# daniabib/ComfyUI_ProPainter_Nodes

Measured on NVIDIA H100. Metric: inpainted frames/sec at 640x360, 80-frame subvideo, higher is better.
Workload: dtype f16

## Files before the change

comfyui_propainter_nodes_b200/csrc/conv_epilogue.cuh:

```cuda
#pragma once
#include "conv_igemm.cuh"
#include "wgmma_ops.cuh"

namespace ppconv {

template <int ACT, bool ACC = false, int N>
__device__ __forceinline__ void act16_t(float (&v)[N], float slope) {
#pragma unroll
  for (int i = 0; i < N; ++i) {
    if (ACT == PP_ACT_RELU) v[i] = fmaxf(v[i], 0.f);
    else if (ACT == PP_ACT_LRELU) v[i] = v[i] > 0.f ? v[i] : v[i] * slope;
    else if (ACT == PP_ACT_SIGMOID) v[i] = ppx::sigmoidf_(v[i]);
    else if (ACT == PP_ACT_TANH) v[i] = ACC ? ppx::tanh_acc(v[i]) : tanhf(v[i]);
    else if (ACT == PP_ACT_GELU) v[i] = ppx::gelu_erf(v[i]);
  }
}
template <bool ACC = false, int N>
__device__ __forceinline__ void act16(float (&v)[N], int act, float slope) {
  switch (act) {
    case PP_ACT_RELU: act16_t<PP_ACT_RELU, ACC>(v, slope); break;
    case PP_ACT_LRELU: act16_t<PP_ACT_LRELU, ACC>(v, slope); break;
    case PP_ACT_SIGMOID: act16_t<PP_ACT_SIGMOID, ACC>(v, slope); break;
    case PP_ACT_TANH: act16_t<PP_ACT_TANH, ACC>(v, slope); break;
    case PP_ACT_GELU: act16_t<PP_ACT_GELU, ACC>(v, slope); break;
    default: break;
  }
}

__device__ __forceinline__ void load16(const __half* src, int nvalid, bool vec, float (&r)[16]) {
  if (vec && nvalid == 16) {
    const uint4 a = reinterpret_cast<const uint4*>(src)[0], b = reinterpret_cast<const uint4*>(src)[1];
    const __half2* ha = reinterpret_cast<const __half2*>(&a);
    const __half2* hb = reinterpret_cast<const __half2*>(&b);
#pragma unroll
    for (int i = 0; i < 4; ++i) {
      const float2 fa = __half22float2(ha[i]), fb = __half22float2(hb[i]);
      r[2 * i] = fa.x; r[2 * i + 1] = fa.y; r[8 + 2 * i] = fb.x; r[8 + 2 * i + 1] = fb.y;
    }
  } else {
#pragma unroll
    for (int i = 0; i < 16; ++i) r[i] = i < nvalid ? __half2float(src[i]) : 0.f;
  }
}
__device__ __forceinline__ void store16(__half* dst, int nvalid, bool vec, const float (&v)[16]) {
  if (vec && nvalid == 16) {
    __align__(16) __half2 h[8];
#pragma unroll
    for (int i = 0; i < 8; ++i) h[i] = __floats2half2_rn(v[2 * i], v[2 * i + 1]);
    reinterpret_cast<uint4*>(dst)[0] = reinterpret_cast<uint4*>(h)[0];
    reinterpret_cast<uint4*>(dst)[1] = reinterpret_cast<uint4*>(h)[1];
  } else {
#pragma unroll
    for (int i = 0; i < 16; ++i)
      if (i < nvalid) dst[i] = __float2half_rn(v[i]);
  }
}

__device__ __forceinline__ void conv_epilogue16(const PPConvParams& p, const uint32_t (&raw)[16], long long mrow, int g,
                                                int ng0, int epi, bool vec) {
    const int nvalid = min(16, p.Cout_g - ng0);
    float v[16];
#pragma unroll
    for (int i = 0; i < 16; ++i) v[i] = __uint_as_float(raw[i]);
    if (p.bias != nullptr) {
      const float* bp = p.bias + g * p.Cout_g + ng0;
      if (vec && nvalid == 16) {
#pragma unroll
        for (int i = 0; i < 4; ++i) {
          const float4 b4 = __ldg(reinterpret_cast<const float4*>(bp) + i);
          v[4 * i] += b4.x; v[4 * i + 1] += b4.y; v[4 * i + 2] += b4.z; v[4 * i + 3] += b4.w;
        }
      } else {
#pragma unroll
        for (int i = 0; i < 16; ++i)
          if (i < nvalid) v[i] += __ldg(bp + i);
      }
    }
    if (epi == PP_EPI_STD) {
      act16(v, p.act1, p.slope);
      if (p.scale != 1.f) {
#pragma unroll
        for (int i = 0; i < 16; ++i) v[i] *= p.scale;
      }
      if (p.aux0 != nullptr) {
        float r[16];
        load16(p.aux0 + mrow * p.aux0_cstride + p.aux0_coff + ng0, nvalid, vec, r);
#pragma unroll
        for (int i = 0; i < 16; ++i) v[i] += r[i];
      }
      act16(v, p.act2, p.slope);
      const long long o = mrow * p.out_cstride + p.out_coff + (long long)g * p.out_gstep + ng0;
      if (p.out_fp32) {
        float* dst = reinterpret_cast<float*>(p.out) + o;
        if (vec && nvalid == 16) {
#pragma unroll
          for (int i = 0; i < 4; ++i)
            reinterpret_cast<float4*>(dst)[i] = make_float4(v[4 * i], v[4 * i + 1], v[4 * i + 2], v[4 * i + 3]);
        } else {
#pragma unroll
          for (int i = 0; i < 16; ++i)
            if (i < nvalid) dst[i] = v[i];
        }
      } else {
        store16(reinterpret_cast<__half*>(p.out) + o, nvalid, vec, v);
      }
    } else if (epi == PP_EPI_GRU_ZR) {
      const int half_c = p.Cout_g >> 1;
      act16_t<PP_ACT_SIGMOID>(v, 0.f);
      if (ng0 < half_c) {
        store16(reinterpret_cast<__half*>(p.out) + mrow * p.out_cstride + p.out_coff + ng0, nvalid, vec, v);
      } else {
        const int c = ng0 - half_c;
        float h[16];
        load16(p.aux0 + mrow * p.aux0_cstride + p.aux0_coff + c, nvalid, vec, h);
#pragma unroll
        for (int i = 0; i < 16; ++i) v[i] *= h[i];
        store16(p.out2 + mrow * p.out2_cstride + p.out2_coff + c, nvalid, vec, v);
      }
    } else {
      float h[16], z[16];
      load16(p.aux0 + mrow * p.aux0_cstride + p.aux0_coff + ng0, nvalid, vec, h);
      load16(p.aux1 + mrow * p.aux1_cstride + p.aux1_coff + ng0, nvalid, vec, z);
      act16_t<PP_ACT_TANH>(v, 0.f);
#pragma unroll
      for (int i = 0; i < 16; ++i) v[i] = (1.f - z[i]) * h[i] + z[i] * v[i];
      store16(reinterpret_cast<__half*>(p.out) + mrow * p.out_cstride + p.out_coff + ng0, nvalid, vec, v);
    }
}


template <int BN>
__device__ __forceinline__ void stage_bias(const PPConvParams& p, float* bs, int goff, int n0, int t128) {
  const int c0 = 2 * t128, n = goff + n0 + c0;
  float2 bv = make_float2(0.f, 0.f);
  if (p.bias != nullptr && c0 < BN) {
    if (n0 + c0 < p.Cout_g) bv.x = __ldg(p.bias + n);
    if (n0 + c0 + 1 < p.Cout_g) bv.y = __ldg(p.bias + n + 1);
  }
  if (c0 < BN) *reinterpret_cast<float2*>(bs + c0) = bv;
}

template <int PW>
__device__ __forceinline__ int frag_stg_off(int r, int c) {
  return r * PW * 2 + ((((c & (PW - 1)) >> 3) ^ ((r * PW * 2 >> 7) & (PW / 8 - 1))) << 4) + (c & 7) * 2;
}

template <int MB, int BN, int PW, int PANEL, int EPI, int ACT1>
__device__ __forceinline__ void frag_epilogue(const PPConvParams& p, const float (&acc)[MB][BN / 2], uint8_t* so,
                                              const uint8_t* zb, const float* bs, bool has_aux, bool r_tile, int P,
                                              int t128) {
  const bool has_bias = p.bias != nullptr;
  const float scale = p.scale, slope = p.slope;
  const int act2 = p.act2;
  const int fr = 16 * (t128 >> 5) + ((t128 & 31) >> 2), fc = 2 * (t128 & 3);
#pragma unroll
  for (int b = 0; b < MB; ++b) {
    const int r = 64 * b + fr;
#pragma unroll
    for (int j = 0; j < BN / 8; ++j) {
      const int col = 8 * j + fc;
      if (EPI == PP_EPI_GRU_H && col / PW != P) continue;
      const int off = (col / PW) * PANEL + frag_stg_off<PW>(r, col);
      __half2* lo = reinterpret_cast<__half2*>(so + off);
      __half2* hi = reinterpret_cast<__half2*>(so + off + 8 * PW * 2);
      const float2 bias = *reinterpret_cast<const float2*>(bs + col);
      float v[4] = {acc[b][4 * j], acc[b][4 * j + 1], acc[b][4 * j + 2], acc[b][4 * j + 3]};
      float a[4] = {0.f, 0.f, 0.f, 0.f};
      if (has_aux) {
        const float2 a0 = __half22float2(*lo), a1 = __half22float2(*hi);
        a[0] = a0.x; a[1] = a0.y; a[2] = a1.x; a[3] = a1.y;
      }
      if (has_bias) {
        v[0] += bias.x; v[1] += bias.y; v[2] += bias.x; v[3] += bias.y;
      }
      if constexpr (EPI == PP_EPI_STD) {
        act16_t<ACT1>(v, slope);
        if (scale != 1.f) {
#pragma unroll
          for (int i = 0; i < 4; ++i) v[i] *= scale;
        }
        if (has_aux) {
#pragma unroll
          for (int i = 0; i < 4; ++i) v[i] += a[i];
        }
        if (act2 != PP_ACT_NONE) act16(v, act2, slope);
      } else if constexpr (EPI == PP_EPI_GRU_ZR) {
        act16_t<PP_ACT_SIGMOID>(v, 0.f);
        if (r_tile) {
#pragma unroll
          for (int i = 0; i < 4; ++i) v[i] *= a[i];
        }
      } else {
        const int zoff = frag_stg_off<PW>(r, col);
        const float2 z0 = __half22float2(*reinterpret_cast<const __half2*>(zb + zoff));
        const float2 z1 = __half22float2(*reinterpret_cast<const __half2*>(zb + zoff + 8 * PW * 2));
        const float z[4] = {z0.x, z0.y, z1.x, z1.y};
        act16_t<PP_ACT_TANH>(v, 0.f);
#pragma unroll
        for (int i = 0; i < 4; ++i) v[i] = (1.f - z[i]) * a[i] + z[i] * v[i];
      }
      *lo = __floats2half2_rn(v[0], v[1]);
      *hi = __floats2half2_rn(v[2], v[3]);
    }
  }
}

__device__ __forceinline__ void load16_split(const float* src, int lo, int nvalid, bool vec, float (&r)[16]) {
  if (vec && nvalid == 16) {
#pragma unroll
    for (int i = 0; i < 4; ++i) {
      const float4 h = reinterpret_cast<const float4*>(src)[i], l = reinterpret_cast<const float4*>(src + lo)[i];
      r[4 * i] = h.x + l.x; r[4 * i + 1] = h.y + l.y; r[4 * i + 2] = h.z + l.z; r[4 * i + 3] = h.w + l.w;
    }
  } else {
#pragma unroll
    for (int i = 0; i < 16; ++i) r[i] = i < nvalid ? src[i] + src[lo + i] : 0.f;
  }
}
__device__ __forceinline__ void store16_split(float* dst, int lo, int nvalid, bool vec, const float (&v)[16]) {
  float h[16], l[16];
#pragma unroll
  for (int i = 0; i < 16; ++i) { h[i] = ppx::tf32_rna(v[i]); l[i] = v[i] - h[i]; }
  if (vec && nvalid == 16) {
#pragma unroll
    for (int i = 0; i < 4; ++i) {
      reinterpret_cast<float4*>(dst)[i] = make_float4(h[4 * i], h[4 * i + 1], h[4 * i + 2], h[4 * i + 3]);
      reinterpret_cast<float4*>(dst + lo)[i] = make_float4(l[4 * i], l[4 * i + 1], l[4 * i + 2], l[4 * i + 3]);
    }
  } else {
#pragma unroll
    for (int i = 0; i < 16; ++i)
      if (i < nvalid) { dst[i] = h[i]; dst[lo + i] = l[i]; }
  }
}

__device__ __forceinline__ void conv_epilogue16_split(const PPConvParams& p, const float (&acc)[16], long long mrow, int g,
                                                      int ng0, bool vec) {
  const int nvalid = min(16, p.Cout_g - ng0);
  float v[16];
#pragma unroll
  for (int i = 0; i < 16; ++i) v[i] = acc[i];
  if (p.bias != nullptr) {
    const float* bp = p.bias + g * p.Cout_g + ng0;
#pragma unroll
    for (int i = 0; i < 16; ++i)
      if (i < nvalid) v[i] += __ldg(bp + i);
  }
  const float* aux0 = reinterpret_cast<const float*>(p.aux0);
  const float* aux1 = reinterpret_cast<const float*>(p.aux1);
  float* out = reinterpret_cast<float*>(p.out);
  if (p.epi == PP_EPI_STD) {
    act16<true>(v, p.act1, p.slope);
    if (p.scale != 1.f) {
#pragma unroll
      for (int i = 0; i < 16; ++i) v[i] *= p.scale;
    }
    if (aux0 != nullptr) {
      float r[16];
      load16_split(aux0 + mrow * p.aux0_cstride + p.aux0_coff + ng0, p.aux0_lo, nvalid, vec, r);
#pragma unroll
      for (int i = 0; i < 16; ++i) v[i] += r[i];
    }
    act16<true>(v, p.act2, p.slope);
    float* dst = out + mrow * p.out_cstride + p.out_coff + (long long)g * p.out_gstep + ng0;
    if (p.out_fp32) {
      if (vec && nvalid == 16) {
#pragma unroll
        for (int i = 0; i < 4; ++i)
          reinterpret_cast<float4*>(dst)[i] = make_float4(v[4 * i], v[4 * i + 1], v[4 * i + 2], v[4 * i + 3]);
      } else {
#pragma unroll
        for (int i = 0; i < 16; ++i)
          if (i < nvalid) dst[i] = v[i];
      }
    } else {
      store16_split(dst, p.out_lo, nvalid, vec, v);
    }
  } else if (p.epi == PP_EPI_GRU_ZR) {
    const int half_c = p.Cout_g >> 1;
    act16_t<PP_ACT_SIGMOID, true>(v, 0.f);
    if (ng0 < half_c) {
      store16_split(out + mrow * p.out_cstride + p.out_coff + ng0, p.out_lo, nvalid, vec, v);
    } else {
      const int c = ng0 - half_c;
      float h[16];
      load16_split(aux0 + mrow * p.aux0_cstride + p.aux0_coff + c, p.aux0_lo, nvalid, vec, h);
#pragma unroll
      for (int i = 0; i < 16; ++i) v[i] *= h[i];
      store16_split(reinterpret_cast<float*>(p.out2) + mrow * p.out2_cstride + p.out2_coff + c, p.out2_lo, nvalid, vec, v);
    }
  } else {
    float h[16], z[16];
    load16_split(aux0 + mrow * p.aux0_cstride + p.aux0_coff + ng0, p.aux0_lo, nvalid, vec, h);
    load16_split(aux1 + mrow * p.aux1_cstride + p.aux1_coff + ng0, p.aux1_lo, nvalid, vec, z);
    act16_t<PP_ACT_TANH, true>(v, 0.f);
#pragma unroll
    for (int i = 0; i < 16; ++i) v[i] = (1.f - z[i]) * h[i] + z[i] * v[i];
    store16_split(out + mrow * p.out_cstride + p.out_coff + ng0, p.out_lo, nvalid, vec, v);
  }
}

constexpr int STG_LD = 40;
constexpr int STG_BYTES = 64 * STG_LD * 4;

template <int N, class Emit>
__device__ __forceinline__ void drain_acc(const float (&acc)[N / 2], float* stg, int t128, int bar_id, Emit&& emit) {
  const int wrow = 16 * (t128 >> 5) + ((t128 & 31) >> 2), wcol = 2 * (t128 & 3);
#pragma unroll 1
  for (int c0 = 0; c0 < N; c0 += 32) {
#pragma unroll
    for (int cc = 0; cc < N; cc += 32) {
      if (cc == c0) {
#pragma unroll
        for (int j = 0; j < 4; ++j) {
          if (cc + 8 * j < N) {
            const int i = (cc / 8 + j) * 4;
            *reinterpret_cast<float2*>(stg + wrow * STG_LD + 8 * j + wcol) = make_float2(acc[i], acc[i + 1]);
            *reinterpret_cast<float2*>(stg + (wrow + 8) * STG_LD + 8 * j + wcol) = make_float2(acc[i + 2], acc[i + 3]);
          }
        }
      }
    }
    ppx::named_bar(bar_id, 128);
    const int c = c0 + 16 * (t128 & 1);
    if (c < N) emit(stg + (t128 >> 1) * STG_LD + 16 * (t128 & 1), t128 >> 1, c);
    ppx::named_bar(bar_id, 128);
  }
}

template <bool SPLIT = false, int EPI = -1>
__device__ __forceinline__ void epilogue_from_stage(const PPConvParams& p, const float* src, long long mrow, int g, int ng0) {
  if constexpr (SPLIT) {
    float acc[16];
#pragma unroll
    for (int i = 0; i < 16; i += 4) {
      const float4 v = *reinterpret_cast<const float4*>(src + i);
      acc[i] = v.x; acc[i + 1] = v.y; acc[i + 2] = v.z; acc[i + 3] = v.w;
    }
// ... 47 lines not shown
```

comfyui_propainter_nodes_b200/csrc/conv_gemm.cu:

```cuda
#include <string.h>

#include "conv_epilogue.cuh"
#include "conv_igemm.cuh"

namespace {

constexpr int NUM_THREADS = 384;
constexpr int NUM_CONSUMERS = 256;
constexpr int WARP_PRODUCER = 8;
constexpr int STAGE_BYTES = 48 * 1024;
constexpr int STAGES = 3;
constexpr int OUT_BYTES = 64 * 1024;
constexpr int BIAS_BYTES = 2 * 256 * 4;
constexpr int SMEM_BYTES = 1024 + STAGES * STAGE_BYTES + OUT_BYTES + 1024 + BIAS_BYTES;

struct GemmParams {
  PPConvParams c;
  CUtensorMap tmap_a[PP_MAX_SEGS];
  CUtensorMap tmap_out;
  CUtensorMap tmap_res;
  int m_tiles, n_tiles, chunks;
  int debug;
};

struct Smem {
  uint8_t* stages;
  uint8_t* out;
  uint64_t *full, *empty, *res;
  float* bias;
};
__device__ __forceinline__ Smem gemm_smem() {
  uint8_t* base = ppx::dyn_smem_1024();
  Smem m;
  m.stages = base;
  m.out = base + STAGES * STAGE_BYTES;
  m.full = reinterpret_cast<uint64_t*>(m.out + OUT_BYTES);
  m.empty = m.full + STAGES;
  m.res = m.empty + STAGES;
  m.bias = reinterpret_cast<float*>(m.out + OUT_BYTES + 1024);
  return m;
}

template <int MB, int BN>
__device__ __forceinline__ void gemm_tile(const GemmParams& h, const Smem& m, int tile, int& s, uint32_t& ph, uint32_t& rph,
                                          int wg, int t128) {
  using namespace ppx;
  const PPConvParams& p = h.c;
  constexpr int A_BYTES = 128 * MB * 128;
  constexpr int WG_ROWS = 64 * MB;
  constexpr int PANEL = 128 * MB * 128;
  const int n0 = (tile % h.n_tiles) * BN;
  const int m0 = (tile / h.n_tiles) * (128 * MB);
  float acc[MB][BN / 2];
  int prev = -1;
  for (int c = 0; c < h.chunks; ++c) {
    mbar_wait(&m.full[s], ph);
    const uint32_t a = smem_u32(m.stages + s * STAGE_BYTES);
    uint64_t adesc[MB];
#pragma unroll
    for (int b = 0; b < MB; ++b) adesc[b] = gmma_desc_sw128_kmajor(a + (wg * MB + b) * 64 * 128);
    const uint64_t bdesc = gmma_desc_sw128_kmajor(a + A_BYTES);
    wgmma_fence();
#pragma unroll
    for (int k = 0; k < 4; ++k)
#pragma unroll
      for (int b = 0; b < MB; ++b) wgmma_f16<BN>(acc[b], adesc[b] + 2 * k, bdesc + 2 * k, (c | k) != 0 ? 1u : 0u);
    wgmma_commit();
    wgmma_wait<1>();
    if (prev >= 0) mbar_arrive(&m.empty[prev]);
    prev = s;
    if (++s == STAGES) { s = 0; ph ^= 1; }
  }
  wgmma_wait<0>();
#pragma unroll
  for (int b = 0; b < MB; ++b) wgmma_fence_acc(acc[b]);
  mbar_arrive(&m.empty[prev]);
  if (h.debug & 1) return;

  const int bar_id = 2 + wg, row0 = m0 + wg * WG_ROWS;
  const int npanel = (min(BN, p.Cout_g - n0) + 63) / 64;
  uint8_t* so = m.out + wg * WG_ROWS * 128;
  const bool issuer = t128 == 0;
  float* bs = m.bias + wg * 256;
  ppconv::stage_bias<BN>(p, bs, 0, n0, t128);
  if (issuer) tma_store_wait_read<0>();
  named_bar(bar_id, 128);
  const bool has_res = p.aux0 != nullptr;
  if (has_res) {
    if (issuer) {
      mbar_arrive_expect_tx(&m.res[wg], (uint32_t)(npanel * WG_ROWS * 128));
      for (int pnl = 0; pnl < npanel; ++pnl) tma_load_2d(smem_u32(so + pnl * PANEL), &h.tmap_res, n0 + pnl * 64, row0, &m.res[wg]);
    }
    mbar_wait(&m.res[wg], rph);
    rph ^= 1;
  }
  auto epilogue = [&](auto act1) {
    ppconv::frag_epilogue<MB, BN, 64, PANEL, PP_EPI_STD, decltype(act1)::value>(p, acc, so, nullptr, bs, has_res, false, 0,
                                                                                t128);
  };
  switch (p.act1) {
    case PP_ACT_RELU: epilogue(ppconv::IntC<PP_ACT_RELU>{}); break;
    case PP_ACT_LRELU: epilogue(ppconv::IntC<PP_ACT_LRELU>{}); break;
    case PP_ACT_SIGMOID: epilogue(ppconv::IntC<PP_ACT_SIGMOID>{}); break;
    case PP_ACT_TANH: epilogue(ppconv::IntC<PP_ACT_TANH>{}); break;
    case PP_ACT_GELU: epilogue(ppconv::IntC<PP_ACT_GELU>{}); break;
    default: epilogue(ppconv::IntC<PP_ACT_NONE>{}); break;
  }
  fence_proxy_async();
  named_bar(bar_id, 128);
  if (issuer) {
    for (int pnl = 0; pnl < npanel; ++pnl) tma_store_2d(&h.tmap_out, smem_u32(so + pnl * PANEL), n0 + pnl * 64, row0);
    tma_store_commit();
  }
}

template <int MB>
__global__ void __launch_bounds__(NUM_THREADS, 1) conv_gemm_kernel(const __grid_constant__ GemmParams h) {
  using namespace ppx;
  constexpr int BN = 256 / MB;
  constexpr int A_BYTES = 128 * MB * 128;
  const Smem m = gemm_smem();
  const PPConvParams& p = h.c;
  const int tid = threadIdx.x, warp = tid >> 5;
  const int total_tiles = h.m_tiles * h.n_tiles;
  if (tid == 0) {
    for (int s = 0; s < STAGES; ++s) { mbar_init(&m.full[s], 1); mbar_init(&m.empty[s], NUM_CONSUMERS); }
    mbar_init(&m.res[0], 1);
    mbar_init(&m.res[1], 1);
    mbar_fence_init();
  }
  __syncthreads();
  asm volatile("griddepcontrol.wait;" ::: "memory");
  asm volatile("griddepcontrol.launch_dependents;" ::: "memory");

  if (warp < 8) setmaxnreg_inc<232>();
  else setmaxnreg_dec<40>();
  if (warp < 8) {
    const int wg = tid >> 7, t128 = tid & 127;
    int s = 0;
    uint32_t ph = 0, rph = 0;
    for (int tile = blockIdx.x; tile < total_tiles; tile += gridDim.x) gemm_tile<MB, BN>(h, m, tile, s, ph, rph, wg, t128);
    if (t128 == 0) tma_store_wait<0>();
  } else if (warp == WARP_PRODUCER) {
    if (elect_one()) {
      int s = 0;
      uint32_t ph = 0;
      for (int tile = blockIdx.x; tile < total_tiles; tile += gridDim.x) {
        const int n0 = (tile % h.n_tiles) * BN;
        const int m0 = (tile / h.n_tiles) * (128 * MB);
        const uint32_t b_bytes = (uint32_t)(min(BN, p.Cout_g_pad - n0) * 128);
        for (int c = 0; c < h.chunks; ++c) {
          const int ci = c * 64;
          const int q = pp_seg_of(p, ci);
          mbar_wait(&m.empty[s], ph ^ 1);
          mbar_arrive_expect_tx(&m.full[s], (uint32_t)A_BYTES + b_bytes);
          const uint32_t dst = smem_u32(m.stages + s * STAGE_BYTES);
          tma_load_4d(dst, &h.tmap_a[q], ci - p.seg[q].cbegin, m0, 0, 0, &m.full[s]);
          bulk_g2s(dst + A_BYTES, p.wpacked + ((long long)c * p.Cout_g_pad + n0) * 64, b_bytes, &m.full[s]);
          if (++s == STAGES) { s = 0; ph ^= 1; }
        }
      }
    }
  }
}

int gemm_mb(const PPConvParams& p) { return p.Cout_g_pad <= 128 && p.M_total >= 256 ? 2 : 1; }

long long gemm_tiles(const PPConvParams& p, int mb) {
  return pp_ceil_div64(p.M_total, 128 * mb) * pp_ceil_div(p.Cout_g_pad, 256 / mb);
}

}

int pp_conv_gemm_eligible(const PPConvParams& p) {
  if (p.kh != 1 || p.kw != 1 || p.sh != 1 || p.sw != 1 || p.ph != 0 || p.pw != 0 || p.pad_replicate) return 0;
  if (p.groups != 1 || p.split || p.epi != PP_EPI_STD || p.out_fp32 || p.M_total < 128) return 0;
  if (!pp_conv_segs_chunked(p, true)) return 0;
  if (!aligned16(p.out, p.out_cstride, p.out_coff)) return 0;
  if (p.aux0 != nullptr && !aligned16(p.aux0, p.aux0_cstride, p.aux0_coff)) return 0;
  if (p.bias != nullptr && (reinterpret_cast<uintptr_t>(p.bias) & 7) != 0) return 0;
  int num_sms = 0;
  if (pp_num_sms(&num_sms) != PP_OK || gemm_tiles(p, gemm_mb(p)) < num_sms) return 0;
  return pp_tmap_supported() ? 1 : 0;
}

int pp_launch_conv_gemm(const PPConvParams& pin, cudaStream_t stream) {
  static bool attr_set = false;
  if (!attr_set) {
    PP_CUDA_CHECK(cudaFuncSetAttribute(conv_gemm_kernel<1>, cudaFuncAttributeMaxDynamicSharedMemorySize, SMEM_BYTES));
    PP_CUDA_CHECK(cudaFuncSetAttribute(conv_gemm_kernel<2>, cudaFuncAttributeMaxDynamicSharedMemorySize, SMEM_BYTES));
    attr_set = true;
  }
  GemmParams h;
  memset(&h, 0, sizeof(h));
  h.c = pin;
  const PPConvParams& p = h.c;
  const int mb = gemm_mb(p);
  h.m_tiles = (int)pp_ceil_div64(p.M_total, 128 * mb);
  h.n_tiles = pp_ceil_div(p.Cout_g_pad, 256 / mb);
  h.chunks = pp_ceil_div(p.Cin, 64);
  PP_REQUIRE((long long)h.m_tiles * h.n_tiles < (1LL << 31), "conv_gemm: too many tiles");
  h.debug = pp_conv_noepi();
  PP_TRY(pp_conv_input_tmaps(p, 128 * mb, 1, true, h.tmap_a));
  PP_TRY(pp_tmap_2d_f16(&h.tmap_out, static_cast<const __half*>(p.out) + p.out_coff, p.Cout_g, p.M_total, p.out_cstride, 64 * mb));
  if (p.aux0 != nullptr)
    PP_TRY(pp_tmap_2d_f16(&h.tmap_res, p.aux0 + p.aux0_coff, p.Cout_g, p.M_total, p.aux0_cstride, 64 * mb));
  int num_sms = 0;
  PP_TRY(pp_num_sms(&num_sms));
  return pp_conv_launch(mb == 2 ? conv_gemm_kernel<2> : conv_gemm_kernel<1>, h, min(h.m_tiles * h.n_tiles, num_sms),
                        NUM_THREADS, SMEM_BYTES, stream);
}
```

comfyui_propainter_nodes_b200/csrc/conv_halo.cu:

```cuda
#include <cuda.h>
#include <stdlib.h>
#include <string.h>

#include <memory>

#include "conv_epilogue.cuh"
#include "conv_igemm.cuh"
#include "dcn_sample.cuh"

namespace {

constexpr int NUM_THREADS = 384;
constexpr int NUM_EPI_THREADS = 256;
constexpr int WARP_A = 8, WARP_B = 9;
constexpr int MAX_SA = 4, MAX_SB = 8;
constexpr int SMEM_BUDGET = 186 * 1024;
constexpr int SMEM_MAX = 227 * 1024;
constexpr int SMEM_ALIGN_SLACK = 1024;
constexpr int BAR_BLOCK_BYTES = 1024;
constexpr int DRAIN_EPI_BYTES = 2 * ppconv::STG_BYTES;

struct HaloLayer {
  PPConvParams c;
  CUtensorMap tmap[PP_MAX_SEGS];
// ... 91 lines not shown
__device__ __forceinline__ void halo_tap_group(int tn, float (&acc)[MB][BN / 2], uint64_t (&adesc)[MB], uint64_t bdesc,
                                               uint32_t& accum, int& kx, int kw, uint32_t step_x, uint32_t step_row,
                                               uint32_t tap16) {
  using namespace ppx;
  if constexpr (NT > 1) {
    if (tn < NT) {
      halo_tap_group<BN, MB, NT - 1, TF32>(tn, acc, adesc, bdesc, accum, kx, kw, step_x, step_row, tap16);
      return;
    }
  }
  wgmma_fence();
#pragma unroll
  for (int tt = 0; tt < NT; ++tt) halo_tap<BN, MB, TF32>(acc, adesc, bdesc, accum, kx, kw, step_x, step_row, tap16);
  wgmma_commit();
}

template <int BN, int MB, int NT, bool TF32, class BeforeWait>
__device__ __forceinline__ void halo_mainloop(const HaloLayer& h, const HaloSmem& m, Ring& ra, Ring& rb, int wg,
                                              float (&acc)[MB][BN / 2], BeforeWait&& before_wait) {
  using namespace ppx;
  const PPConvParams& p = h.c;
  const int taps = p.kh * p.kw;
  const uint32_t sbo = h.flat ? 1024u : (uint32_t)h.BW * 128;
  const uint32_t step_x = (uint32_t)p.dw * 8;
  const uint32_t step_row = (uint32_t)(p.dh * h.BW - (p.kw - 1) * p.dw) * 8;
  const uint32_t tap16 = (uint32_t)p.BN * 8;
  const int kw = p.kw;
  uint32_t aoff[MB];
#pragma unroll
  for (int b = 0; b < MB; ++b) aoff[b] = MB == 2 ? wg * h.sub_bytes + b * 8 * sbo : wg * 8 * sbo;
  uint32_t accum = 0;
  int pend_a = -1, pend_b = -1;
  for (int c = 0; c < h.chunks; ++c) {
    mbar_wait(&m.a_full[ra.s], ra.ph);
    uint64_t adesc[MB];
#pragma unroll
    for (int b = 0; b < MB; ++b) adesc[b] = gmma_desc_sw128_kmajor(smem_u32(m.a + ra.s * m.a_stage_bytes) + aoff[b], sbo);
    int kx = 0;
    for (int tap0 = 0; tap0 < taps; tap0 += h.tps) {
      mbar_wait(&m.b_full[rb.s], rb.ph);
      const uint64_t bdesc = gmma_desc_sw128_kmajor(smem_u32(m.b + rb.s * m.b_stage_bytes));
      halo_tap_group<BN, MB, NT, TF32>(min(h.tps, taps - tap0), acc, adesc, bdesc, accum, kx, kw, step_x, step_row, tap16);
      wgmma_wait<1>();
      if (pend_b >= 0) mbar_arrive(&m.b_empty[pend_b]);
      if (pend_a >= 0) mbar_arrive(&m.a_empty[pend_a]);
      pend_b = rb.s;
      pend_a = tap0 + h.tps >= taps ? ra.s : -1;
      if (++rb.s == m.SB) { rb.s = 0; rb.ph ^= 1; }
    }
    if (++ra.s == m.SA) { ra.s = 0; ra.ph ^= 1; }
  }
  before_wait();
  wgmma_wait<0>();
#pragma unroll
  for (int b = 0; b < MB; ++b) wgmma_fence_acc(acc[b]);
  if (pend_b >= 0) mbar_arrive(&m.b_empty[pend_b]);
  if (pend_a >= 0) mbar_arrive(&m.a_empty[pend_a]);
}

template <int BN, int MB, int NT, bool TF32 = false, bool PROG = false>
__device__ __forceinline__ void halo_tile(const HaloLayer& h, int tile, const HaloSmem& m, Ring& ra, Ring& rb, float* stg,
                                          int wg, int t128) {
  const PPConvParams& p = h.c;
  const TileCoord t = decode_tile(h, tile);
  const int n0 = t.n_idx * p.BN;
  const int bnt = min(p.BN, p.Cout_g_pad - n0);
  float acc[MB][BN / 2];
  halo_mainloop<BN, MB, NT, TF32>(h, m, ra, rb, wg, acc, [] {});

  const bool skip = (h.debug & 1) != 0;
#pragma unroll
  for (int b = 0; b < MB; ++b) {
    const int sub = MB == 2 ? wg : 0, rbase = MB == 2 ? 64 * b : 64 * wg;
    ppconv::drain_acc<BN>(acc[b], stg, t128, 4 + wg, [&](const float* src, int r64, int cc) {
      const int r = rbase + r64;
      bool mvalid;
      long long mrow;
      if (h.flat) {
        mrow = ((long long)t.tx * h.MT + sub) * 128 + r;
        mvalid = mrow < p.M_total;
      } else {
        const int oy = t.ty * 16 + (r >> 3), ox = t.tx * (8 * h.MT) + 8 * sub + (r & 7);
        mvalid = oy < p.OH && ox < p.OW;
        mrow = ((long long)t.img * p.OH + oy) * p.OW + ox;
      }
      if (!mvalid || skip || cc >= bnt || n0 + cc >= p.Cout_g) return;
      ppconv::epilogue_from_stage<TF32, PROG ? PP_EPI_STD : -1>(p, src, mrow, t.g, n0 + cc);
    });
  }
}

__host__ __device__ constexpr int halo_panel_width(int bn) { return bn % 64 == 0 ? 64 : bn % 32 == 0 ? 32 : 16; }
__host__ __device__ constexpr int halo_out_stage_bytes(int mt, int bn) { return 2 * 64 * mt * bn * 2; }
__host__ __device__ constexpr int halo_out_bias_bytes(int bn) { return (2 * bn * 4 + 1023) / 1024 * 1024; }
__host__ __device__ constexpr int halo_out_z_bytes(int mt, int bn) { return 2 * 64 * mt * halo_panel_width(bn) * 2; }
__host__ __device__ constexpr int halo_tma_region_bytes(int mt, int bn, bool gru_h) {
  return halo_out_stage_bytes(mt, bn) + halo_out_bias_bytes(bn) + (gru_h ? halo_out_z_bytes(mt, bn) : 0);
}
__host__ __device__ inline int halo_epi_bytes(const HaloParams& h) {
  return h.tma_out ? halo_tma_region_bytes(h.MT, h.c.BN, h.c.epi == PP_EPI_GRU_H) : DRAIN_EPI_BYTES;
}
__device__ __forceinline__ uint64_t* halo_out_bar(const HaloSmem& m, int wg) { return m.spare + 1 + wg; }

template <int BN, int MB, int NT>
__device__ __forceinline__ void halo_tile_tma(const HaloParams& h, int tile, const HaloSmem& m, Ring& ra, Ring& rb,
                                              uint32_t& xph, int wg, int t128) {
  using namespace ppx;
  const PPConvParams& p = h.c;
  constexpr int PW = halo_panel_width(BN);
  constexpr int PANEL = 64 * MB * PW * 2;
  const TileCoord t = decode_tile(h, tile);
  const int n0 = t.n_idx * BN;
  const int epi = p.epi;
  const int half_c = p.Cout_g >> 1;
  const bool r_tile = epi == PP_EPI_GRU_ZR && n0 >= half_c;
  const bool has_aux = epi == PP_EPI_STD ? p.aux0 != nullptr : (epi == PP_EPI_GRU_H || r_tile);
  const int npanel = (min(BN, p.Cout_g - n0) + PW - 1) / PW;
  uint8_t* so = m.epi + wg * (64 * MB * BN * 2);
  float* bs = reinterpret_cast<float*>(m.epi + halo_out_stage_bytes(MB, BN)) + wg * BN;
  uint8_t* zb = m.epi + halo_out_stage_bytes(MB, BN) + halo_out_bias_bytes(BN) + wg * PANEL;
  uint64_t* xbar = halo_out_bar(m, wg);
  int x0, y0, img;
  if (h.flat) {
    x0 = MB == 2 ? (t.tx * 2 + wg) * 128 : t.tx * 128 + 64 * wg; y0 = 0; img = 0;
  } else {
    x0 = t.tx * (8 * MB) + (MB == 2 ? 8 * wg : 0); y0 = t.ty * 16 + (MB == 2 ? 0 : 8 * wg); img = t.img;
  }
  const int aux_c = r_tile ? n0 - half_c : n0;
  const bool issuer = t128 == 0;
  const bool skip = (h.debug & 1) != 0;
  float acc[MB][BN / 2];
  halo_mainloop<BN, MB, NT, false>(h, m, ra, rb, wg, acc, [&] {
    if (issuer && has_aux && !skip) {
      tma_store_wait_read<0>();
      const int nz = epi == PP_EPI_GRU_H ? 1 : 0;
      mbar_arrive_expect_tx(xbar, (uint32_t)((npanel + nz) * PANEL));
      for (int pn = 0; pn < npanel; ++pn)
        tma_load_4d(smem_u32(so + pn * PANEL), &h.tm_aux0, aux_c + pn * PW, x0, y0, img, xbar);
      if (nz) tma_load_4d(smem_u32(zb), &h.tm_aux1, n0, x0, y0, img, xbar);
    }
  });
  if (skip) return;

  ppconv::stage_bias<BN>(p, bs, t.g * p.Cout_g, n0, t128);
  const int bar_id = 4 + wg;
  if (issuer && !has_aux) tma_store_wait_read<0>();
  named_bar(bar_id, 128);
  if (has_aux) {
    mbar_wait(xbar, xph);
    xph ^= 1;
  }
  using ppconv::IntC;
  auto epilogue = [&](auto kind, auto act1, bool aux, int P) {
    ppconv::frag_epilogue<MB, BN, PW, PANEL, decltype(kind)::value, decltype(act1)::value>(p, acc, so, zb, bs, aux, r_tile,
                                                                                           P, t128);
  };
  if (epi == PP_EPI_STD) {
    switch (p.act1) {
      case PP_ACT_RELU: epilogue(IntC<PP_EPI_STD>{}, IntC<PP_ACT_RELU>{}, has_aux, 0); break;
      case PP_ACT_LRELU: epilogue(IntC<PP_EPI_STD>{}, IntC<PP_ACT_LRELU>{}, has_aux, 0); break;
      default: epilogue(IntC<PP_EPI_STD>{}, IntC<PP_ACT_NONE>{}, has_aux, 0); break;
    }
  } else if (epi == PP_EPI_GRU_ZR) {
    epilogue(IntC<PP_EPI_GRU_ZR>{}, IntC<PP_ACT_NONE>{}, r_tile, 0);
  } else {
#pragma unroll 1
    for (int pn = 0; pn < npanel; ++pn) {
      if (pn > 0) {
        named_bar(bar_id, 128);
        if (issuer) {
          mbar_arrive_expect_tx(xbar, (uint32_t)PANEL);
          tma_load_4d(smem_u32(zb), &h.tm_aux1, n0 + pn * PW, x0, y0, img, xbar);
        }
        mbar_wait(xbar, xph);
        xph ^= 1;
      }
      epilogue(IntC<PP_EPI_GRU_H>{}, IntC<PP_ACT_NONE>{}, true, pn);
    }
  }
  fence_proxy_async();
  named_bar(bar_id, 128);
  if (issuer) {
    const CUtensorMap* tm = r_tile ? &h.tm_out2 : &h.tm_out;
    const int c0 = r_tile ? n0 - half_c : t.g * p.out_gstep + n0;
    for (int pn = 0; pn < npanel; ++pn) tma_store_4d(tm, smem_u32(so + pn * PANEL), c0 + pn * PW, x0, y0, img);
    tma_store_commit();
  }
}

template <class F>
__device__ __forceinline__ void with_tile_shape(int mt, int bn, F&& f) {
  if (mt == 2) ppconv::with_tile_width<128>(bn, [&](auto n) { f(n, ppconv::IntC<2>{}); });
  else ppconv::with_tile_width<256>(bn, [&](auto n) { f(n, ppconv::IntC<1>{}); });
}

__device__ __forceinline__ void halo_smem_init_barriers(const HaloSmem& m) {
  using namespace ppx;
  for (int s = 0; s < m.SA; ++s) { mbar_init(&m.a_full[s], 1); mbar_init(&m.a_empty[s], NUM_EPI_THREADS); }
  for (int s = 0; s < m.SB; ++s) { mbar_init(&m.b_full[s], 1); mbar_init(&m.b_empty[s], NUM_EPI_THREADS); }
  mbar_fence_init();
}

__device__ __forceinline__ void halo_produce_patches(const HaloLayer& h, const HaloSmem& m, Ring& r) {
  using namespace ppx;
  const PPConvParams& p = h.c;
  const int total_tiles = halo_total_tiles(h);
  const uint32_t bytes = (uint32_t)(h.BW * h.BH * 128);
  for (int tile = blockIdx.x; tile < total_tiles; tile += gridDim.x) {
    const TileCoord t = decode_tile(h, tile);
    const int x0 = h.flat ? t.tx * (128 * h.MT) : t.tx * (8 * h.MT) - p.pw, y0 = h.flat ? 0 : t.ty * 16 - p.ph;
    for (int c = 0; c < h.chunks; ++c) {
      const int ci = c * 64;
      const int q = pp_seg_of(p, ci);
      const int ch0 = t.g * p.seg[q].gstep + (ci - p.seg[q].cbegin);
      mbar_wait(&m.a_empty[r.s], r.ph ^ 1);
      mbar_arrive_expect_tx(&m.a_full[r.s], bytes);
      tma_load_4d(smem_u32(m.a + r.s * m.a_stage_bytes), &h.tmap[q], ch0, x0, y0, t.img, &m.a_full[r.s]);
      if (++r.s == m.SA) { r.s = 0; r.ph ^= 1; }
    }
  }
}

__device__ __forceinline__ void halo_produce_weights(const HaloLayer& h, const HaloSmem& m, Ring& r) {
  using namespace ppx;
  const PPConvParams& p = h.c;
  const int total_tiles = halo_total_tiles(h);
  const int taps = p.kh * p.kw;
  for (int tile = blockIdx.x; tile < total_tiles; tile += gridDim.x) {
    const TileCoord t = decode_tile(h, tile);
    const int n0 = t.n_idx * p.BN;
    const uint32_t bytes = (uint32_t)(min(p.BN, p.Cout_g_pad - n0) * 128);
    const __half* wbase = p.wpacked + ((long long)t.g * p.num_kc * p.Cout_g_pad + n0) * 64;
    for (int c = 0; c < h.chunks; ++c) {
      for (int tap0 = 0; tap0 < taps; tap0 += h.tps) {
        const int tn = min(h.tps, taps - tap0);
        mbar_wait(&m.b_empty[r.s], r.ph ^ 1);
        mbar_arrive_expect_tx(&m.b_full[r.s], bytes * (uint32_t)tn);
        for (int t = 0; t < tn; ++t) {
          const int kc = (tap0 + t) * h.chunks + c;
          bulk_g2s(smem_u32(m.b + r.s * m.b_stage_bytes + t * p.BN * 128), wbase + (long long)kc * p.Cout_g_pad * 64, bytes,
                   &m.b_full[r.s]);
        }
        if (++r.s == m.SB) { r.s = 0; r.ph ^= 1; }
      }
    }
  }
}

template <bool TF32>
__device__ __forceinline__ void halo_body(const HaloParams& h) {
  using namespace ppx;
  const HaloSmem m = halo_smem(dyn_smem_1024(), h.SA, h.a_stage_bytes, h.SB, h.b_stage_bytes, halo_epi_bytes(h));
  const int tid = threadIdx.x, warp = tid >> 5;
  if (tid == 0) {
    if constexpr (!TF32) {
      mbar_init(halo_out_bar(m, 0), 1);
      mbar_init(halo_out_bar(m, 1), 1);
    }
    halo_smem_init_barriers(m);
  }
  __syncthreads();
  asm volatile("griddepcontrol.wait;" ::: "memory");
  asm volatile("griddepcontrol.launch_dependents;" ::: "memory");

  if (warp < 8) setmaxnreg_inc<232>();
  else setmaxnreg_dec<40>();
  if (warp < 8) {
    const int wg = tid >> 7, t128 = tid & 127;
    float* stg = reinterpret_cast<float*>(m.epi + wg * ppconv::STG_BYTES);
    Ring ra = {0, 0}, rb = {0, 0};
    const int total_tiles = halo_total_tiles(h);
    if constexpr (!TF32) {
      if (h.tma_out) {
        uint32_t xph = 0;
        with_tile_shape(h.MT, h.c.BN, [&](auto bn, auto mb) {
          constexpr int BN = decltype(bn)::value;
          for (int tile = blockIdx.x; tile < total_tiles; tile += gridDim.x)
            halo_tile_tma<BN, decltype(mb)::value, halo_max_tps(BN)>(h, tile, m, ra, rb, xph, wg, t128);
        });
        if (t128 == 0) tma_store_wait<0>();
        return;
      }
    }
    with_tile_shape(h.MT, h.c.BN, [&](auto bn, auto mb) {
      constexpr int BN = decltype(bn)::value;
      for (int tile = blockIdx.x; tile < total_tiles; tile += gridDim.x)
        halo_tile<BN, decltype(mb)::value, halo_max_tps(BN), TF32>(h, tile, m, ra, rb, stg, wg, t128);
    });
  } else if (warp == WARP_A) {
    if (elect_one()) {
      Ring r = {0, 0};
      halo_produce_patches(h, m, r);
    }
  } else if (warp == WARP_B) {
    if (elect_one()) {
      Ring r = {0, 0};
      halo_produce_weights(h, m, r);
    }
  }
}

__global__ void __launch_bounds__(NUM_THREADS, 1) conv_halo_kernel(const __grid_constant__ HaloParams h) {
  halo_body<false>(h);
}

__global__ void __launch_bounds__(NUM_THREADS, 1) conv_halo_tf32_kernel(const __grid_constant__ HaloParams h) {
  halo_body<true>(h);
}
// ... 384 lines not shown
```

Baseline: 184.5.

## Give each GEMM warpgroup its own tile to overlap epilogue with the other's MMA

Restructures the persistent 1x1-conv GEMM so the two consumer warpgroups process alternating tiles (64*MB rows each) instead of splitting one tile. An mma_done barrier serialises their main loops so one warpgroup's epilogue and TMA store can overlap the other's WGMMA. Per-MB shared-memory plans give MB=2 five stages, and MB=2 is now always chosen unless an env var forces MB=1. The epilogue also gets a compile-time path for act2==NONE to drop the runtime activation switch. Risks include smaller per-warpgroup tiles lowering B reuse and forcing MB=2 for shapes that previously used MB=1.

Result: faster. 190.7, median of 6 (+3.4%).

```diff
diff --git a/comfyui_propainter_nodes_b200/csrc/conv_epilogue.cuh b/comfyui_propainter_nodes_b200/csrc/conv_epilogue.cuh
--- a/comfyui_propainter_nodes_b200/csrc/conv_epilogue.cuh
+++ b/comfyui_propainter_nodes_b200/csrc/conv_epilogue.cuh
@@ -145,7 +145,7 @@
   return r * PW * 2 + ((((c & (PW - 1)) >> 3) ^ ((r * PW * 2 >> 7) & (PW / 8 - 1))) << 4) + (c & 7) * 2;
 }
 
-template <int MB, int BN, int PW, int PANEL, int EPI, int ACT1>
+template <int MB, int BN, int PW, int PANEL, int EPI, int ACT1, int ACT2 = -1>
 __device__ __forceinline__ void frag_epilogue(const PPConvParams& p, const float (&acc)[MB][BN / 2], uint8_t* so,
                                               const uint8_t* zb, const float* bs, bool has_aux, bool r_tile, int P,
                                               int t128) {
@@ -183,7 +183,8 @@
 #pragma unroll
           for (int i = 0; i < 4; ++i) v[i] += a[i];
         }
-        if (act2 != PP_ACT_NONE) act16(v, act2, slope);
+        if constexpr (ACT2 >= 0) act16_t<ACT2>(v, slope);
+        else if (act2 != PP_ACT_NONE) act16(v, act2, slope);
       } else if constexpr (EPI == PP_EPI_GRU_ZR) {
         act16_t<PP_ACT_SIGMOID>(v, 0.f);
         if (r_tile) {
diff --git a/comfyui_propainter_nodes_b200/csrc/conv_gemm.cu b/comfyui_propainter_nodes_b200/csrc/conv_gemm.cu
--- a/comfyui_propainter_nodes_b200/csrc/conv_gemm.cu
+++ b/comfyui_propainter_nodes_b200/csrc/conv_gemm.cu
@@ -1,3 +1,4 @@
+#include <stdlib.h>
 #include <string.h>
 
 #include "conv_epilogue.cuh"
@@ -6,13 +7,26 @@
 namespace {
 
 constexpr int NUM_THREADS = 384;
-constexpr int NUM_CONSUMERS = 256;
+constexpr int WG_THREADS = 128;
 constexpr int WARP_PRODUCER = 8;
-constexpr int STAGE_BYTES = 48 * 1024;
-constexpr int STAGES = 3;
-constexpr int OUT_BYTES = 64 * 1024;
-constexpr int BIAS_BYTES = 2 * 256 * 4;
-constexpr int SMEM_BYTES = 1024 + STAGES * STAGE_BYTES + OUT_BYTES + 1024 + BIAS_BYTES;
+constexpr int OUT_BYTES = 32 * 1024;
+constexpr int BAR_BYTES = 128;
+
+template <int MB>
+struct Plan {
+  static constexpr int BN = 256 / MB;
+  static constexpr int WG_ROWS = 64 * MB;
+  static constexpr int A_BYTES = WG_ROWS * 128;
+  static constexpr int STAGE_BYTES = A_BYTES + BN * 128;
+  static constexpr int STAGES = MB == 1 ? 3 : 5;
+  static constexpr int OUT_OFF = STAGES * STAGE_BYTES;
+  static constexpr int BIAS_OFF = OUT_OFF + 2 * OUT_BYTES;
+  static constexpr int BAR_OFF = BIAS_OFF + 2 * BN * 4;
+  static constexpr int SMEM_BYTES = 1024 + BAR_OFF + BAR_BYTES;
+  static_assert((2 * STAGES + 4) * 8 <= BAR_BYTES, "conv_gemm: barrier block too small");
+  static_assert(SMEM_BYTES <= 227 * 1024, "conv_gemm: shared-memory plan exceeds 227 KB");
+  static_assert((BN / 64) * A_BYTES == OUT_BYTES, "conv_gemm: staging tile is one warpgroup's tile");
+};
 
 struct GemmParams {
   PPConvParams c;
@@ -26,40 +40,45 @@
 struct Smem {
   uint8_t* stages;
   uint8_t* out;
-  uint64_t *full, *empty, *res;
+  uint64_t *full, *empty, *res, *mma_done;
   float* bias;
 };
+template <int MB>
 __device__ __forceinline__ Smem gemm_smem() {
   uint8_t* base = ppx::dyn_smem_1024();
+  constexpr int STAGES = Plan<MB>::STAGES;
   Smem m;
   m.stages = base;
-  m.out = base + STAGES * STAGE_BYTES;
-  m.full = reinterpret_cast<uint64_t*>(m.out + OUT_BYTES);
+  m.out = base + Plan<MB>::OUT_OFF;
+  m.bias = reinterpret_cast<float*>(base + Plan<MB>::BIAS_OFF);
+  m.full = reinterpret_cast<uint64_t*>(base + Plan<MB>::BAR_OFF);
   m.empty = m.full + STAGES;
   m.res = m.empty + STAGES;
-  m.bias = reinterpret_cast<float*>(m.out + OUT_BYTES + 1024);
+  m.mma_done = m.res + 2;
   return m;
 }
 
-template <int MB, int BN>
-__device__ __forceinline__ void gemm_tile(const GemmParams& h, const Smem& m, int tile, int& s, uint32_t& ph, uint32_t& rph,
-                                          int wg, int t128) {
+template <int MB>
+__device__ __forceinline__ void gemm_tile(const GemmParams& h, const Smem& m, int tile, int it, uint32_t& rph, int wg,
+                                          int t128) {
   using namespace ppx;
+  using P = Plan<MB>;
+  constexpr int BN = P::BN, WG_ROWS = P::WG_ROWS;
+  constexpr int PANEL = WG_ROWS * 128;
   const PPConvParams& p = h.c;
-  constexpr int A_BYTES = 128 * MB * 128;
-  constexpr int WG_ROWS = 64 * MB;
-  constexpr int PANEL = 128 * MB * 128;
   const int n0 = (tile % h.n_tiles) * BN;
-  const int m0 = (tile / h.n_tiles) * (128 * MB);
+  const int m0 = (tile / h.n_tiles) * WG_ROWS;
   float acc[MB][BN / 2];
+  int s = it % P::STAGES;
+  uint32_t ph = (uint32_t)(it / P::STAGES) & 1u;
   int prev = -1;
   for (int c = 0; c < h.chunks; ++c) {
     mbar_wait(&m.full[s], ph);
-    const uint32_t a = smem_u32(m.stages + s * STAGE_BYTES);
+    const uint32_t a = smem_u32(m.stages + s * P::STAGE_BYTES);
     uint64_t adesc[MB];
 #pragma unroll
-    for (int b = 0; b < MB; ++b) adesc[b] = gmma_desc_sw128_kmajor(a + (wg * MB + b) * 64 * 128);
-    const uint64_t bdesc = gmma_desc_sw128_kmajor(a + A_BYTES);
+    for (int b = 0; b < MB; ++b) adesc[b] = gmma_desc_sw128_kmajor(a + b * 64 * 128);
+    const uint64_t bdesc = gmma_desc_sw128_kmajor(a + P::A_BYTES);
     wgmma_fence();
 #pragma unroll
     for (int k = 0; k < 4; ++k)
@@ -69,34 +88,39 @@
     wgmma_wait<1>();
     if (prev >= 0) mbar_arrive(&m.empty[prev]);
     prev = s;
-    if (++s == STAGES) { s = 0; ph ^= 1; }
-  }
+    if (++s == P::STAGES) { s = 0; ph ^= 1; }
+  }
+  mbar_arrive(&m.mma_done[wg]);
   wgmma_wait<0>();
 #pragma unroll
   for (int b = 0; b < MB; ++b) wgmma_fence_acc(acc[b]);
   mbar_arrive(&m.empty[prev]);
   if (h.debug & 1) return;
 
-  const int bar_id = 2 + wg, row0 = m0 + wg * WG_ROWS;
+  const int bar_id = 2 + wg;
   const int npanel = (min(BN, p.Cout_g - n0) + 63) / 64;
-  uint8_t* so = m.out + wg * WG_ROWS * 128;
+  uint8_t* so = m.out + wg * OUT_BYTES;
   const bool issuer = t128 == 0;
-  float* bs = m.bias + wg * 256;
+  float* bs = m.bias + wg * BN;
   ppconv::stage_bias<BN>(p, bs, 0, n0, t128);
   if (issuer) tma_store_wait_read<0>();
-  named_bar(bar_id, 128);
+  named_bar(bar_id, WG_THREADS);
   const bool has_res = p.aux0 != nullptr;
   if (has_res) {
     if (issuer) {
-      mbar_arrive_expect_tx(&m.res[wg], (uint32_t)(npanel * WG_ROWS * 128));
-      for (int pnl = 0; pnl < npanel; ++pnl) tma_load_2d(smem_u32(so + pnl * PANEL), &h.tmap_res, n0 + pnl * 64, row0, &m.res[wg]);
+      mbar_arrive_expect_tx(&m.res[wg], (uint32_t)(npanel * PANEL));
+      for (int pnl = 0; pnl < npanel; ++pnl) tma_load_2d(smem_u32(so + pnl * PANEL), &h.tmap_res, n0 + pnl * 64, m0, &m.res[wg]);
     }
     mbar_wait(&m.res[wg], rph);
     rph ^= 1;
   }
   auto epilogue = [&](auto act1) {
-    ppconv::frag_epilogue<MB, BN, 64, PANEL, PP_EPI_STD, decltype(act1)::value>(p, acc, so, nullptr, bs, has_res, false, 0,
-                                                                                t128);
+    if (p.act2 == PP_ACT_NONE)
+      ppconv::frag_epilogue<MB, BN, 64, PANEL, PP_EPI_STD, decltype(act1)::value, PP_ACT_NONE>(p, acc, so, nullptr, bs, has_res,
+                                                                                             false, 0, t128);
+    else
+      ppconv::frag_epilogue<MB, BN, 64, PANEL, PP_EPI_STD, decltype(act1)::value>(p, acc, so, nullptr, bs, has_res, false, 0,
+                                                                                  t128);
   };
   switch (p.act1) {
     case PP_ACT_RELU: epilogue(ppconv::IntC<PP_ACT_RELU>{}); break;
@@ -107,9 +131,9 @@
     default: epilogue(ppconv::IntC<PP_ACT_NONE>{}); break;
   }
   fence_proxy_async();
-  named_bar(bar_id, 128);
+  named_bar(bar_id, WG_THREADS);
   if (issuer) {
-    for (int pnl = 0; pnl < npanel; ++pnl) tma_store_2d(&h.tmap_out, smem_u32(so + pnl * PANEL), n0 + pnl * 64, row0);
+    for (int pnl = 0; pnl < npanel; ++pnl) tma_store_2d(&h.tmap_out, smem_u32(so + pnl * PANEL), n0 + pnl * 64, m0);
     tma_store_commit();
   }
 }
@@ -117,16 +141,14 @@
 template <int MB>
 __global__ void __launch_bounds__(NUM_THREADS, 1) conv_gemm_kernel(const __grid_constant__ GemmParams h) {
   using namespace ppx;
-  constexpr int BN = 256 / MB;
-  constexpr int A_BYTES = 128 * MB * 128;
-  const Smem m = gemm_smem();
+  using P = Plan<MB>;
+  const Smem m = gemm_smem<MB>();
   const PPConvParams& p = h.c;
   const int tid = threadIdx.x, warp = tid >> 5;
   const int total_tiles = h.m_tiles * h.n_tiles;
   if (tid == 0) {
-    for (int s = 0; s < STAGES; ++s) { mbar_init(&m.full[s], 1); mbar_init(&m.empty[s], NUM_CONSUMERS); }
-    mbar_init(&m.res[0], 1);
-    mbar_init(&m.res[1], 1);
+    for (int s = 0; s < P::STAGES; ++s) { mbar_init(&m.full[s], 1); mbar_init(&m.empty[s], WG_THREADS); }
+    for (int w = 0; w < 2; ++w) { mbar_init(&m.res[w], 1); mbar_init(&m.mma_done[w], WG_THREADS); }
     mbar_fence_init();
   }
   __syncthreads();
@@ -137,37 +159,47 @@
   else setmaxnreg_dec<40>();
   if (warp < 8) {
     const int wg = tid >> 7, t128 = tid & 127;
-    int s = 0;
-    uint32_t ph = 0, rph = 0;
-    for (int tile = blockIdx.x; tile < total_tiles; tile += gridDim.x) gemm_tile<MB, BN>(h, m, tile, s, ph, rph, wg, t128);
+    uint32_t rph = 0;
+    int j = wg;
+    for (int tile = blockIdx.x + wg * gridDim.x; tile < total_tiles; tile += 2 * gridDim.x, j += 2) {
+      if (j > 0) mbar_wait(&m.mma_done[wg ^ 1], (uint32_t)((j - 1) >> 1) & 1u);
+      gemm_tile<MB>(h, m, tile, j * h.chunks, rph, wg, t128);
+    }
     if (t128 == 0) tma_store_wait<0>();
   } else if (warp == WARP_PRODUCER) {
     if (elect_one()) {
       int s = 0;
       uint32_t ph = 0;
       for (int tile = blockIdx.x; tile < total_tiles; tile += gridDim.x) {
-        const int n0 = (tile % h.n_tiles) * BN;
-        const int m0 = (tile / h.n_tiles) * (128 * MB);
-        const uint32_t b_bytes = (uint32_t)(min(BN, p.Cout_g_pad - n0) * 128);
+        const int n0 = (tile % h.n_tiles) * P::BN;
+        const int m0 = (tile / h.n_tiles) * P::WG_ROWS;
+        const uint32_t b_bytes = (uint32_t)(min(P::BN, p.Cout_g_pad - n0) * 128);
         for (int c = 0; c < h.chunks; ++c) {
           const int ci = c * 64;
           const int q = pp_seg_of(p, ci);
           mbar_wait(&m.empty[s], ph ^ 1);
-          mbar_arrive_expect_tx(&m.full[s], (uint32_t)A_BYTES + b_bytes);
-          const uint32_t dst = smem_u32(m.stages + s * STAGE_BYTES);
+          mbar_arrive_expect_tx(&m.full[s], (uint32_t)P::A_BYTES + b_bytes);
+          const uint32_t dst = smem_u32(m.stages + s * P::STAGE_BYTES);
           tma_load_4d(dst, &h.tmap_a[q], ci - p.seg[q].cbegin, m0, 0, 0, &m.full[s]);
-          bulk_g2s(dst + A_BYTES, p.wpacked + ((long long)c * p.Cout_g_pad + n0) * 64, b_bytes, &m.full[s]);
-          if (++s == STAGES) { s = 0; ph ^= 1; }
+          bulk_g2s(dst + P::A_BYTES, p.wpacked + ((long long)c * p.Cout_g_pad + n0) * 64, b_bytes, &m.full[s]);
+          if (++s == P::STAGES) { s = 0; ph ^= 1; }
         }
       }
     }
   }
 }
 
-int gemm_mb(const PPConvParams& p) { return p.Cout_g_pad <= 128 && p.M_total >= 256 ? 2 : 1; }
+int gemm_mb(const PPConvParams&) {
+  static int forced = -1;
+  if (forced < 0) {
+    const char* e = getenv("PP_GEMM_MB");
+    forced = e != nullptr ? atoi(e) : 0;
+  }
+  return forced == 1 ? 1 : 2;
+}
 
 long long gemm_tiles(const PPConvParams& p, int mb) {
-  return pp_ceil_div64(p.M_total, 128 * mb) * pp_ceil_div(p.Cout_g_pad, 256 / mb);
+  return pp_ceil_div64(p.M_total, 64 * mb) * pp_ceil_div(p.Cout_g_pad, 256 / mb);
 }
 
 }
@@ -187,8 +219,8 @@
 int pp_launch_conv_gemm(const PPConvParams& pin, cudaStream_t stream) {
   static bool attr_set = false;
   if (!attr_set) {
-    PP_CUDA_CHECK(cudaFuncSetAttribute(conv_gemm_kernel<1>, cudaFuncAttributeMaxDynamicSharedMemorySize, SMEM_BYTES));
-    PP_CUDA_CHECK(cudaFuncSetAttribute(conv_gemm_kernel<2>, cudaFuncAttributeMaxDynamicSharedMemorySize, SMEM_BYTES));
+    PP_CUDA_CHECK(cudaFuncSetAttribute(conv_gemm_kernel<1>, cudaFuncAttributeMaxDynamicSharedMemorySize, Plan<1>::SMEM_BYTES));
+    PP_CUDA_CHECK(cudaFuncSetAttribute(conv_gemm_kernel<2>, cudaFuncAttributeMaxDynamicSharedMemorySize, Plan<2>::SMEM_BYTES));
     attr_set = true;
   }
   GemmParams h;
@@ -196,17 +228,17 @@
   h.c = pin;
   const PPConvParams& p = h.c;
   const int mb = gemm_mb(p);
-  h.m_tiles = (int)pp_ceil_div64(p.M_total, 128 * mb);
+  h.m_tiles = (int)pp_ceil_div64(p.M_total, 64 * mb);
   h.n_tiles = pp_ceil_div(p.Cout_g_pad, 256 / mb);
   h.chunks = pp_ceil_div(p.Cin, 64);
   PP_REQUIRE((long long)h.m_tiles * h.n_tiles < (1LL << 31), "conv_gemm: too many tiles");
   h.debug = pp_conv_noepi();
-  PP_TRY(pp_conv_input_tmaps(p, 128 * mb, 1, true, h.tmap_a));
+  PP_TRY(pp_conv_input_tmaps(p, 64 * mb, 1, true, h.tmap_a));
   PP_TRY(pp_tmap_2d_f16(&h.tmap_out, static_cast<const __half*>(p.out) + p.out_coff, p.Cout_g, p.M_total, p.out_cstride, 64 * mb));
   if (p.aux0 != nullptr)
     PP_TRY(pp_tmap_2d_f16(&h.tmap_res, p.aux0 + p.aux0_coff, p.Cout_g, p.M_total, p.aux0_cstride, 64 * mb));
   int num_sms = 0;
   PP_TRY(pp_num_sms(&num_sms));
   return pp_conv_launch(mb == 2 ? conv_gemm_kernel<2> : conv_gemm_kernel<1>, h, min(h.m_tiles * h.n_tiles, num_sms),
-                        NUM_THREADS, SMEM_BYTES, stream);
-}
+                        NUM_THREADS, mb == 2 ? Plan<2>::SMEM_BYTES : Plan<1>::SMEM_BYTES, stream);
+}
diff --git a/comfyui_propainter_nodes_b200/csrc/conv_halo.cu b/comfyui_propainter_nodes_b200/csrc/conv_halo.cu
--- a/comfyui_propainter_nodes_b200/csrc/conv_halo.cu
+++ b/comfyui_propainter_nodes_b200/csrc/conv_halo.cu
@@ -267,8 +267,11 @@
   }
   using ppconv::IntC;
   auto epilogue = [&](auto kind, auto act1, bool aux, int P) {
-    ppconv::frag_epilogue<MB, BN, PW, PANEL, decltype(kind)::value, decltype(act1)::value>(p, acc, so, zb, bs, aux, r_tile,
-                                                                                           P, t128);
+    constexpr int KIND = decltype(kind)::value, ACT1 = decltype(act1)::value;
+    if (KIND == PP_EPI_STD && p.act2 == PP_ACT_NONE)
+      ppconv::frag_epilogue<MB, BN, PW, PANEL, KIND, ACT1, PP_ACT_NONE>(p, acc, so, zb, bs, aux, r_tile, P, t128);
+    else
+      ppconv::frag_epilogue<MB, BN, PW, PANEL, KIND, ACT1>(p, acc, so, zb, bs, aux, r_tile, P, t128);
   };
   if (epi == PP_EPI_STD) {
     switch (p.act1) {
```
